# ChristophReich1996/Multi-StyleGAN

Measured on AMD Instinct MI355X. Metric: training images/sec (G+D step, 256^2, seq=3x2ch), higher is better.
Workload: dtype bf16

## Files before the change

include/msg_hip.h:

```cpp
#ifndef MSG_HIP_H
#define MSG_HIP_H

#ifdef __cplusplus
extern "C" {
#endif

enum { MSG_OK = 0, MSG_EINVAL = -1, MSG_EUNSUPPORTED = -2, MSG_ELAUNCH = -3 };
enum { MSG_F32 = 0, MSG_BF16 = 1, MSG_F16 = 2, MSG_F64 = 3, MSG_F32_SPLIT = 4 };

#define MSG_ABI_VERSION 5
int msg_abi_version(void);
const char* msg_build_arch(void);
const char* msg_strerror(int code);

int msg_upfirdn2d(const void* x, const float* fir, void* y, int dtype,
                  int major, int in_h, int in_w, int minor, int kh, int kw,
                  int up_x, int up_y, int down_x, int down_y,
                  int pad_x0, int pad_x1, int pad_y0, int pad_y1, void* stream);

int msg_upfirdn2d_pitched(const void* x, const float* fir, void* y, int dtype,
                          int major, int in_h, int in_w, int minor, int in_pitch, int kh, int kw,
                          int up_x, int up_y, int down_x, int down_y,
                          int pad_x0, int pad_x1, int pad_y0, int pad_y1, void* stream);

// ... 119 lines not shown

long long msg_minibatch_stddev_workspace(int C, int H, int W, int groups, int dtype);
int msg_minibatch_stddev(const void* x, void* y, float* stat, float* workspace, int dtype,
                         int B, int C, int H, int W, int ldx, int ldy, int groups, float alpha, void* stream);
int msg_minibatch_stddev_backward(const void* x, const void* gy, const float* gstat, void* gx, int dtype,
                                  int B, int C, int H, int W, int ldx, int ldgy, int ldgx, int groups,
                                  float alpha, void* stream);

int msg_conv2d_fprop_act(const void* x, const void* w, void* y, int dtype,
                         int B, int IH, int IW, int Cx, int Ck, int OH, int OW, int N, int ldy,
                         int kh, int kw, int stride, int pad, long long w_batch_stride,
                         const float* act_bias, const float* noise, const float* noise_weight,
                         int noise_batch, float alpha, float scale, void* stream);
int msg_conv2d_fprop_act_mask(const void* x, const void* w, void* y, int dtype,
                              int B, int IH, int IW, int Cx, int Ck, int OH, int OW, int N, int ldy,
                              int kh, int kw, int stride, int pad, long long w_batch_stride,
                              const float* act_bias, const float* noise, const float* noise_weight,
                              int noise_batch, float alpha, float scale, unsigned char* mask, void* stream);

int msg_conv2d_fprop_residual(const void* x, const void* w, void* y, int dtype,
                              int B, int IH, int IW, int Cx, int Ck, int OH, int OW, int N, int ldy,
                              int kh, int kw, int stride, int pad, long long w_batch_stride,
                              const void* residual, int res_ld, float gain, void* stream);

long long msg_conv2d_fprop_act_backward_workspace(int dtype, int B, int IH, int IW, int Cx, int Ck, int OH, int OW,
                                                  int N, int kh, int kw, long long w_batch_stride, int has_noise);
int msg_conv2d_fprop_act_backward(const void* x, const void* w, void* y, int dtype,
                                  int B, int IH, int IW, int Cx, int Ck, int OH, int OW, int N, int ldy,
                                  int kh, int kw, int stride, int pad, long long w_batch_stride,
                                  const void* residual, int res_ld,
                                  const unsigned char* sign_mask, int mask_tile_m, int mask_tile_n,
                                  const void* sign_map, int sign_ld, float alpha, float scale,
                                  float* grad_bias, const float* noise, int noise_batch, float* grad_noise_weight,
                                  float* ws, long long ws_floats, void* stream);

int msg_act_pointwise_head(const void* x, const float* bias, const float* w, float* y, int dtype,
                           long long npix, int C, float wscale, float alpha, float scale, void* stream);
long long msg_act_pointwise_head_backward_workspace(long long npix, int C);
int msg_act_pointwise_head_backward(const void* x, const float* bias, const float* w, const float* gy, void* gx,
                                    float* grad_bias_and_w, int dtype, long long npix, int C, float wscale,
                                    float alpha, float scale, float* ws, long long ws_floats, void* stream);

int msg_linear_fprop(const float* x, const float* w, const float* bias, float* y, int M, int N, int K,
                     float gain, float bias_gain, void* stream);
int msg_linear_dgrad(const float* gy, const float* w, float* gx, int M, int N, int K, float gain, void* stream);
int msg_linear_wgrad(const float* gy, const float* x, float* gw, float* gb, int M, int N, int K,
// ... 66 lines not shown
```

multi_stylegan_amd/conv_ops.py:

```python
import math
import os
from typing import Optional, Tuple

import torch
from torch.autograd import Function

from . import _lib
from ._autograd import _derive


def _vec(dtype) -> int:
    return 8 if dtype == torch.bfloat16 else 4


def _round_up(n: int, m: int) -> int:
    return (n + m - 1) // m * m


def _padded_nhwc(b, c, h, w, dtype, device):
    cx = _round_up(c, _vec(dtype))
    buf = torch.empty((b, h, w, cx), dtype=dtype, device=device)
    if cx != c:
        buf[..., c:].zero_()
    return buf.permute(0, 3, 1, 2)[:, :c]
# ... 390 lines not shown
            act_bias, noise, noise_w, alpha, scale = act[:5]
            _lib.require_gpu(x, act_bias, noise, noise_w)
            mask = None
            if len(act) > 5 and act[5] is not None and kh == 3 and stride == 1 and pad == 1:
                pkey = (x.dtype, b, ih, iw, cx, ck, oh, ow, n, kh, kw, wstride)
                mplan = _PLAN_CACHE.get(pkey)
                if mplan is None:
                    mplan = _PLAN_CACHE[pkey] = _lib.lib().msg_conv2d_fprop_plan(_lib.dtype_code(x), b, ih, iw, cx, ck, oh, ow,
                                                                                n, kh, kw, wstride)
                tile = _PLANS[mplan][1]
                if tile:
                    from .op_static.fused_act import sign_mask_for
                    mask = sign_mask_for(b, n, oh, ow, x.dtype, dev)
                    if mask is not None:
                        act[5].append((mask, tile, tile))
            code = _lib.lib().msg_conv2d_fprop_act_mask(
                xv.data_ptr(), wk.data_ptr(), y.data_ptr(), _contraction_code(x, mode), b, ih, iw, cx, ck, oh, ow, n, ldy, kh, kw,
                stride, pad, wstride, _lib.ptr(act_bias), _lib.ptr(noise), _lib.ptr(noise_w),
                1 if noise is None else noise.shape[0], float(alpha), float(scale), _lib.ptr(mask), _lib.stream_of(dev))
    _lib.check(code, "msg_conv2d_fprop")
    return y


def _grad_dest(param):
    if param is None or "_msg_grad_slot" not in getattr(param, "__dict__", ()):
        return None
    from .dist import grad_destination
    return grad_destination(param)


def wgrad_k_chunks(b, o, i, taps, oh, ow, per_sample, kp):
    tiles = ((o + 127) // 128) * ((i + 127) // 128) * taps * b
    if per_sample:
        return max(1, min((oh * ow) // (16 * kp), 1024 // tiles)) if tiles < 256 else 1
    k_chunks = max(1, min((oh * ow + 4 * kp - 1) // (4 * kp), (1024 + tiles - 1) // tiles))
    while b * k_chunks > 65535:
        k_chunks -= 1
    return k_chunks


def _launch_wgrad(gy, x, o, i, kh, kw, stride, pad, pixel_shuffle, per_sample, low_hw, raw=False, gain=1.0, out=None,
                  mode=None):
    dev = _lib.require_gpu(gy, x)
    gv, ldgy = _nhwc_view(gy)
    xv, cx = _nhwc_view(x)
    b, _, ih, iw = xv.shape
# ... 212 lines not shown
            _lib.ptr(gb), _lib.ptr(nz), nb, _lib.ptr(gnw), ws, need, _lib.stream_of(dev))
    if code == _lib.MSG_EUNSUPPORTED:
        _ACTBWD_WS_CACHE[wkey] = 0
        return None
    _lib.check(code, "msg_conv2d_fprop_act_backward")
    handle.done = (gb, gnw)
    return y


def _d_raw(gy, w, g: Geometry, residual=None, act_bwd: Optional["ActHandle"] = None, sign_map=None):
    if act_bwd is not None and act_bwd.armed and not g.per_sample and g.kind == "conv" and g.stride == 1 and g.kh == 3 and \
            g.kw == 3 and g.pad == 1 and w.ndim == 4:
        i = _oi(w)[1]
        img = _param_images(w, gy.dtype, g.wscale, g.kind)
        wk, ok = img["d"] if img is not None else \
            _cached(w, "d" + g.kind, gy.dtype, g.wscale, lambda: _relay_dgrad(w, gy.dtype, flip=True))
        out = _launch_dgrad_act_backward(gy, wk, ok, i, 3, 3, False, _oi(w)[0], act_bwd, residual=residual, mode=g.mode,
                                         sign_map=sign_map)
        if out is not None:
            return out
    return _d_raw_plain(gy, w, g, residual)


def _d_raw_plain(gy, w, g: Geometry, residual=None):
    assert residual is None or (g.kind == "conv" and g.stride == 1)
    if g.kind == "conv" and g.stride == 2 and _oi(w)[1] % _vec(gy.dtype) == 0:
        return _d_raw_s2(gy, w, g)
    i = _oi(w)[1]
    if w.ndim == 4 and _thin_ok(gy.dtype, i, g) and i <= 8 and gy.shape[1] >= 64:
        return _d_raw_thin(gy, w, g, residual)
    img = _param_images(w, gy.dtype, g.wscale, g.kind) if not g.per_sample else None
    wk, ok = img["d"] if img is not None else \
        _cached(w, "d" + g.kind, gy.dtype, g.wscale, lambda: _relay_dgrad(w, gy.dtype, flip=g.kind != "up2"))
    if g.kind == "up2":
        return _launch_fprop(gy, wk, ok, None, i, g.x_hw, 2, 2, 2, 0, 1, False, g.per_sample, _oi(w)[0], mode=g.mode)
    pad = g.kh - 1 - g.pad
    assert g.kh == g.kw
    return _launch_fprop(gy, wk, ok, None, i, g.x_hw, g.kh, g.kw, 1, pad, g.stride, False, g.per_sample, _oi(w)[0],
                         residual=residual, mode=g.mode)


def _relay_thin_dgrad(w, dtype):
    o, i, kh, kw = w.shape
    esz = 2 if dtype == torch.bfloat16 else 4
    ko, ok = 128 // esz, _round_up(o, 128 // esz)
    out = torch.zeros((ko, 1, ok), dtype=dtype, device=w.device)
# ... 152 lines not shown
            return gw.unsqueeze(0)
        return gw.reshape(oi) if w_ndim == 2 else gw

    @staticmethod
    def backward(ctx, u):
        gy, x = ctx.saved_tensors
        g = ctx.g
        ggy = _derive(_ConvF, x, u, None, g) if ctx.needs_input_grad[0] else None
        gx = _derive(_ConvD, gy, u, g) if ctx.needs_input_grad[1] else None
        return ggy, gx, None, None, None, None


class _ConvActF(Function):

    @staticmethod
    def forward(ctx, x, w, act_bias, noise, noise_w, g, alpha, scale, slot=None, out_scale=None, act_handle=None,
                input_act=None):
        o = _oi(w)[0]
        b32, nz, nw = _act_operands(act_bias, noise, noise_w, (x.shape[0], o, *g.y_hw))
        holder = [] if any(ctx.needs_input_grad) else None
        y = _f_raw(x, w, None, g, act=(b32, nz, nw, alpha, scale, holder))
        ctx.mask = holder[0] if holder else None
        ctx.slot, ctx.out_scale = slot, out_scale
        ctx.act_handle = ctx.input_act = None
        if act_handle is not None and out_scale is None and noise is None and holder is not None:
            act_handle.arm(y, ctx.mask, alpha, scale, act_bias, act_bias is not None, None)
            ctx.act_handle = act_handle if act_handle.armed else None
        if input_act is not None and input_act.armed:
            ctx.input_act = input_act
        ctx.bias_param = act_bias
        ctx.g, ctx.cfg = g, (alpha, scale, act_bias is not None, noise is not None)
        ctx.nw_shape = None if noise_w is None else noise_w.shape
        ctx.save_for_backward(x, w, y, noise)
        return y

    @staticmethod
    def backward(ctx, gy):
        from .op_static.fused_act import FusedLeakyReLUFunctionBackward
        x, w, y, noise = ctx.saved_tensors
        alpha, scale, has_bias, has_noise = ctx.cfg
        g = ctx.g
        owed = 1.0
        if ctx.out_scale is not None and ctx.out_scale.pending is not None:
            owed, ctx.out_scale.pending = ctx.out_scale.pending, None
        handed = ctx.act_handle.done if ctx.act_handle is not None else None
        if handed is not None:
            ctx.act_handle.done = None
            gpre, (gb, gnw) = gy, handed
        else:
            gpre, gb, gnw = _derive(FusedLeakyReLUFunctionBackward, gy, y, noise if has_noise else None,
                                    ctx.bias_param if has_bias else False, alpha, scale * owed, ctx.mask)
        gx = None
        if ctx.needs_input_grad[0]:
            other = ctx.slot.g if ctx.slot is not None else None
            pre = ctx.input_act if not torch.is_grad_enabled() else None
            if _dgrad_add_ok(other, x.shape, gpre.dtype, g):
                gx = _derive(_ConvD, gpre, w, g, other) if torch.is_grad_enabled() else \
                    _d_raw(gpre, w, g, residual=(other, 1.0), act_bwd=pre, sign_map=x)
                ctx.slot.merged = True
            elif pre is not None:
                gx = _d_raw(gpre, w, g, act_bwd=pre, sign_map=x)
            else:
                gx = _derive(_ConvD, gpre, w, g)
        gw = _derive(_ConvG, gpre, x, _oi(w), w.ndim, g, w) if _consumed(ctx, 1, 1) else None
        return gx, gw, (gb if has_bias and ctx.needs_input_grad[2] else None), None, \
            (gnw.reshape(ctx.nw_shape) if has_noise and ctx.needs_input_grad[4] else None), None, None, None, None, None, None, None


class _ConvResidualF(Function):

    @staticmethod
    def forward(ctx, x, w, main, g, gain, fork, slot=None, main_scale=None, out=None):
        y = _f_raw(x, w, None, g, residual=(main, gain), out=out)
        if out is not None:
            y = out.view_as(out)
        ctx.slot, ctx.main_scale = slot, main_scale
        ctx.g, ctx.gain, ctx.fork = g, float(gain), fork
        ctx.save_for_backward(x, w)
        return (y, y.view_as(y)) if fork else y

    @staticmethod
    def backward(ctx, *grads):
        from .op_static.fused_act import _ScaledAddRows, _rows_ok
        x, w = ctx.saved_tensors
        g1 = grads[0]
        g2 = grads[1] if ctx.fork else None
        if (g1 is None or g2 is None) and ctx.main_scale is not None and ctx.needs_input_grad[2]:
            gs = g1 if g1 is not None else g2
            ctx.main_scale.pending = ctx.gain
            gg = Geometry(ctx.g.kind, ctx.g.kh, ctx.g.kw, ctx.g.stride, ctx.g.pad, ctx.g.x_hw, ctx.g.per_sample,
                          ctx.g.wscale * ctx.gain, mode=ctx.g.mode)
            gs_main = gs
            if torch.is_grad_enabled() and ctx.needs_input_grad[0] and RESIDUAL_FORK_NODE:
                gx, gs_main = _ConvDFork.apply(gs, w, gg)
            else:
                gx = _derive(_ConvD, gs, w, gg) if ctx.needs_input_grad[0] else None
            if ctx.slot is not None and gx is not None:
                ctx.slot.g = gx
            gw = _derive(_ConvG, gs, x, _oi(w), w.ndim, gg, w) if _consumed(ctx, 1, 1) else None
            return gx, gw, gs_main, None, None, None, None, None, None
        if g1 is None or g2 is None:
            gs = (g1 if g1 is not None else g2) * ctx.gain
        elif _rows_ok(g1, g2):
            gs = _derive(_ScaledAddRows, g1, g2, ctx.gain)
        else:
            gs = (g1 + g2) * ctx.gain
        gx = _derive(_ConvD, gs, w, ctx.g) if ctx.needs_input_grad[0] else None
        if ctx.slot is not None and gx is not None:
            ctx.slot.g = gx
        gw = _derive(_ConvG, gs, x, _oi(w), w.ndim, ctx.g, w) if _consumed(ctx, 1, 1) else None
        return gx, gw, (gs if ctx.needs_input_grad[2] else None), None, None, None, None, None, None


class _MultiConvF(Function):

    @staticmethod
    def forward(ctx, x, geoms, *weights):
        ctx.geoms = geoms
        ctx.save_for_backward(x, *weights)
        return tuple(_f_raw(x, w, None, g) for w, g in zip(weights, geoms))

    @staticmethod
    def backward(ctx, *grads):
        x, *weights = ctx.saved_tensors
        second_order = torch.is_grad_enabled()
        gx, gws = None, []
        for k, (gy, w, g) in enumerate(zip(grads, weights, ctx.geoms)):
            if gy is None:
                gws.append(None)
                continue
# ... 3 lines not shown
                    gx = part if gx is None else gx + part
                elif second_order:
                    gx = _derive(_ConvD, gy, w, g, gx)
                else:
                    gx = _d_raw(gy, w, g, residual=(gx, 1.0))
            gws.append(_derive(_ConvG, gy, x, _oi(w), w.ndim, g, w) if _consumed(ctx, 2 + k, 1 + k) else None)
        return (gx, None, *gws)


def conv2d_shared_input(x, weights_and_scales, padding=0):
    p = _square(padding, "padding")
    geoms = tuple(Geometry("conv", w.shape[2], w.shape[3], 1, p, x.shape[2:], False, ws) for w, ws in weights_and_scales)
    return _MultiConvF.apply(x, geoms, *[w for w, _ in weights_and_scales])


class GradScale:
    __slots__ = ("pending",)

    def __init__(self):
        self.pending = None


class GradSlot:
    __slots__ = ("g", "merged")

    def __init__(self):
        self.g, self.merged = None, False


class HeadGradSlot:
    __slots__ = ("head", "dgrad", "armed")

    def __init__(self):
        self.head = None
        self.dgrad = None
        self.armed = False

    def take(self):
        head, dgrad, self.head, self.dgrad = self.head, self.dgrad, None, None
        return head, dgrad


class _ForkInput(Function):

    @staticmethod
    def forward(ctx, x, slot):
        ctx.slot = slot
        return x.view_as(x), x.view_as(x)

    @staticmethod
    def backward(ctx, g_main, g_res):
        slot = ctx.slot
        merged, slot.g, slot.merged = slot.merged, None, False
        if merged or g_res is None:
            return g_main, None
        if g_main is None:
            return g_res, None
        return g_main + g_res, None


def _square(value, what: str) -> int:
    if isinstance(value, int):
        return value
    value = tuple(value)
    if len(value) != 2 or value[0] != value[1]:
        raise _lib.MsgHipError(f"conv2d: only square {what} is implemented, got {value}")
    return int(value[0])


def fork_input(x, slot: GradSlot):
    return _ForkInput.apply(x, slot)


def conv2d_add_residual(x, weight, main, gain, stride=1, padding=0, wscale=1.0, fork=False, grad_slot=None,
                        main_grad_scale=None, out=None):
    s, p = _square(stride, "stride"), _square(padding, "padding")
# ... 670 lines not shown
```

multi_stylegan_amd/csrc/conv_dispatch.h:

```cpp
#pragma once
#include "msg_common.h"

struct ConvProblem {
    int dtype;
    int split;
    int B, IH, IW, Cx, Ck, OH, OW, N, ldy;
    int kh, kw, stride, pad, in_up, pixel_shuffle;
    long long w_batch_stride;

    bool per_sample() const { return w_batch_stride != 0; }
    int samples() const { return per_sample() ? B : 1; }
    long long mtot() const { return per_sample() ? (long long)OH * OW : (long long)B * OH * OW; }
    int esz() const { return dtype == MSG_BF16 ? 2 : 4; }
    long long x_bstride() const { return (long long)IH * IW * Cx; }
    long long y_bstride() const { return (pixel_shuffle ? 4ll : 1ll) * OH * OW * ldy; }
    long long x_bytes() const { return (long long)(per_sample() ? 1 : B) * IH * IW * Cx * esz(); }
    long long w_bytes() const { return (long long)N * kh * kw * Ck * esz(); }
    bool fits31() const { return x_bytes() < 0x7ffffff0ll && w_bytes() < 0x7ffffff0ll; }
};

enum ConvKernel {
    CONV_THIN_N, CONV_THIN_K,
    CONV_UPCONV,
    CONV_ROW3, CONV_ROW3N,
// ... 14 lines not shown
    p.B = q.B; p.IH = q.IH; p.IW = q.IW; p.Cx = q.Cx; p.Ck = q.Ck; p.OH = q.OH; p.OW = q.OW; p.N = q.N; p.ldy = q.ldy;
    p.per_sample = q.per_sample();
    if (act) p.act = *act;
    p.x_bstride = q.x_bstride();
    p.w_bstride = q.w_batch_stride;
    p.y_bstride = q.y_bstride();
    p.Mtot = (int)q.mtot();
}
template <typename P>
inline void conv_fill_taps(P& p, const ConvProblem& q) {
    p.kh = q.kh; p.kw = q.kw; p.stride = q.stride; p.pad = q.pad; p.in_up = q.in_up; p.pixel_shuffle = q.pixel_shuffle;
}

ConvPlan conv_fprop_select(const ConvProblem& q, const ActEpilogue* act, bool has_bias);

bool conv_thin_eligible(const ConvProblem& q, const ActEpilogue* act, ConvPlan* plan);
void conv_thin_launch(const ConvProblem& q, const ConvPlan& plan, const void* x, const void* w, const float* bias, void* y,
                      const ActEpilogue* act, void* stream);
bool conv_upconv_eligible(const ConvProblem& q, const ActEpilogue* act, bool has_bias, ConvPlan* plan);
void conv_upconv_launch(const ConvProblem& q, const ConvPlan& plan, const void* x, const void* w, void* y, void* stream);
bool conv_row3_eligible(const ConvProblem& q, const ActEpilogue* act, bool has_bias, ConvPlan* plan);
void conv_row3_launch(const ConvProblem& q, const ConvPlan& plan, const void* x, const void* w, const float* bias, void* y,
                      const ActEpilogue* act, void* stream);
bool conv_pp_eligible(const ConvProblem& q, ConvPlan* plan);
void conv_pp_launch(const ConvProblem& q, const ConvPlan& plan, const void* x, const void* w, const float* bias, void* y,
                    const ActEpilogue* act, void* stream);

struct WgradProblem {
    int dtype, split;
    int B, IH, IW, Cx, I, OH, OW, ldgy, O, ldgw;
    int kh, kw, stride, pad, pixel_shuffle;
    int per_sample, k_chunks, oi_major;
    float gain;
    int esz() const { return dtype == MSG_BF16 ? 2 : 4; }
    long long gy_bytes() const { return (long long)(pixel_shuffle ? 4 : 1) * OH * OW * ldgy * esz(); }
    long long x_bytes() const { return (long long)IH * IW * Cx * esz(); }
    long long slab() const { return (long long)O * kh * kw * ldgw; }
    long long gw_zstride() const { return oi_major ? (long long)O * I * kh * kw : slab(); }
};

enum WgradKernel {
    WGRAD_GENERIC, WGRAD_DMA, WGRAD_UNI,
    WGRAD_ROW3, WGRAD_ROW3_W32
};

struct WgradPlan {
// ... 27 lines not shown
```

multi_stylegan_amd/csrc/conv_fprop.hip:

```cpp
#include "conv_dispatch.h"
#include <stdlib.h>

typedef __bf16 bf16v8 __attribute__((ext_vector_type(8)));
typedef const __attribute__((address_space(1))) char* gptr_t;
typedef const __attribute__((address_space(1))) u32x4* gvec_t;
typedef __attribute__((address_space(3))) char* lds_t;

struct ConvParams {
    int B, IH, IW, Cx, Ck, OH, OW, N, ldy;
    int kh, kw, stride, pad, in_up, pixel_shuffle, per_sample;
    long long x_bstride, w_bstride, y_bstride;
    int Mtot, n_chunks, n_iters, m_tiles, n_tiles;
    ActEpilogue act;
};

constexpr int BM = 128, BN = 128, ROWB = 128;
constexpr int STAGE_BYTES = (BM + BN) * ROWB;
__device__ __attribute__((aligned(256))) unsigned int g_zero_page[16384];

__device__ __forceinline__ int swz(int row, int slot) { return row * ROWB + ((slot ^ ((row >> 1) & 7)) << 4); }

template <int SPLIT>
__device__ __forceinline__ void split_park(const u32x4& raw, char* dst) {
    uint2 pl[3];
// ... 562 lines not shown
static int conv2d_fprop_impl(const void* x, const void* w, const float* bias, void* y, const ConvProblem& q,
                             const ActEpilogue& act, void* stream, const ConvPlan* selected) {
    if (q.B == 0) return MSG_OK;
    if (!x || !w || !y || q.B < 0 || q.IH <= 0 || q.IW <= 0 || q.OH <= 0 || q.OW <= 0 || q.N <= 0 || q.kh <= 0 || q.kw <= 0 ||
        q.stride <= 0 || q.in_up <= 0 || q.Cx <= 0 || q.Ck <= 0 || q.ldy <= 0)
        return MSG_EINVAL;
    if (q.dtype != MSG_F32 && q.dtype != MSG_BF16) return MSG_EUNSUPPORTED;
    const int vec = 16 / q.esz(), bke = ROWB / q.esz();
    if (q.Ck % bke || q.Cx % vec || (((uintptr_t)x | (uintptr_t)w | (uintptr_t)y) & 15u)) return MSG_EUNSUPPORTED;
    if (q.ldy % vec || (q.pixel_shuffle && (q.N % 4 || (q.N / 4) % vec))) return MSG_EUNSUPPORTED;
    if (q.in_up > 1 && q.stride != 1) return MSG_EUNSUPPORTED;
    const ConvPlan plan = selected ? *selected : conv_fprop_select(q, &act, bias != nullptr);
    if (!plan.supported) return MSG_EUNSUPPORTED;
    switch (plan.kernel) {
        case CONV_THIN_N: case CONV_THIN_K: conv_thin_launch(q, plan, x, w, bias, y, &act, stream); break;
        case CONV_UPCONV: conv_upconv_launch(q, plan, x, w, y, stream); break;
        case CONV_ROW3: case CONV_ROW3N: conv_row3_launch(q, plan, x, w, bias, y, &act, stream); break;
        case CONV_PP: conv_pp_launch(q, plan, x, w, bias, y, &act, stream); break;
        case CONV_DMA: case CONV_REG: case CONV_REG_LEAN: case CONV_REG_SPLIT:
            conv_generic_launch(q, plan, x, w, bias, y, &act, stream); break;
    }
    return MSG_CHECK_LAUNCH();
}
```

multi_stylegan_amd/csrc/conv_fprop_row3.hip:

```cpp
#include "conv_dispatch.h"
#include <stdlib.h>
#include <type_traits>

typedef __bf16 bf16v8 __attribute__((ext_vector_type(8)));
typedef __attribute__((address_space(3))) char* lds_t;

struct ConvParamsR3 {
    int B, IH, IW, Cx, Ck, OH, OW, N, ldy;
    int per_sample, seg_len, n_seg;
    long long x_bstride, w_bstride, y_bstride;
    int Mtot, n_chunks, n_iters, m_tiles, n_tiles;
    int seg_magic;
    int ow_shift, ohw_shift;
    ActEpilogue act;
};

constexpr int HROW = 128;
constexpr int H_OOB = (int)0x80000000;

#ifdef MSG_ROW3_STAMPS
__device__ unsigned long long g_row3_stamps[256 * 4 * 3 * 8];
#define R3_STAMP(k) do { if (it >= 9 && it < 12 && L + 256 >= gridDim.x && blockIdx.z == gridDim.z - 1 && lane == 0) { unsigned long long tt; \
    asm volatile("s_memtime %0\n\ts_waitcnt lgkmcnt(0)" : "=s"(tt) :: "memory"); \
    g_row3_stamps[(((L + 256 - gridDim.x) * 4 + wid_u) * 3 + (it - 9)) * 8 + (k)] = tt; } } while (0)
extern "C" int msg_row3_debug_read(void* host_dst, int nbytes) {
    return hipMemcpyFromSymbol(host_dst, HIP_SYMBOL(g_row3_stamps), nbytes) == hipSuccess ? 0 : -1;
}
__device__ unsigned long long g_row3_clock[256 * 4 * 8];
#define R3_CLOCK(k) do { if (L + 256 >= gridDim.x && blockIdx.z == gridDim.z - 1 && lane == 0) { unsigned long long tc, tr; \
    const unsigned cl_ = L + 256 - gridDim.x; \
    asm volatile("s_memtime %0\n\ts_memrealtime %1\n\ts_waitcnt lgkmcnt(0)" : "=s"(tc), "=s"(tr) :: "memory"); \
    g_row3_clock[(cl_ * 4 + wid_u) * 8 + 2 * (k)] = tc; g_row3_clock[(cl_ * 4 + wid_u) * 8 + 2 * (k) + 1] = tr; } } while (0)
extern "C" int msg_row3_clock_read(void* host_dst, int nbytes) {
    return hipMemcpyFromSymbol(host_dst, HIP_SYMBOL(g_row3_clock), nbytes) == hipSuccess ? 0 : -1;
}
#else
#define R3_STAMP(k) do {} while (0)
#define R3_CLOCK(k) do {} while (0)
#endif

template <int MI, int NCOLB, bool S16, int EPI = 0>
__global__ __launch_bounds__(256, MI == 2 ? 2 : 1) void conv_fprop_row3_kernel(const bf16_t* __restrict__ x, const bf16_t* __restrict__ w,
                                                                 bf16_t* __restrict__ y, const float* __restrict__ bias,
                                                                 ConvParamsR3 p) {
    constexpr int VEC = 8, ESZ = 2;
    constexpr int HN = 64 * NCOLB, HB = HN * HROW, WN = 32 * NCOLB;
    constexpr int NBP = 2 * NCOLB;
    constexpr int HM = 64 * MI, WM = 32 * MI;
    constexpr int NAP = 2 * MI;
    constexpr int HA = (HM + 8) * HROW;
#if defined(MSG_ROW3_NO_STAGGER)
    constexpr bool STAGGER = false;
#else
    constexpr bool STAGGER = true;
#endif
    constexpr int EP_OFF = 2 * HA + 2 * HB;
    constexpr int SIGN_OFF = EP_OFF + (HM + HN) * 4;
    __shared__ __attribute__((aligned(16))) char smem[SIGN_OFF + (EPI == 1 ? HM * (HN / 8) : 0)];
    float* const ep_noise = reinterpret_cast<float*>(smem + EP_OFF);
    float* const ep_bias = ep_noise + HM;

    const int tid = threadIdx.x, lane = tid & 63, wid = tid >> 6;
    const int wid_u = __builtin_amdgcn_readfirstlane(wid);
    const int wm = wid_u >> 1, wn = wid_u & 1;
    constexpr int BLK = S16 ? 16 : 32;
    constexpr int NSUB = S16 ? 2 : 4, SLOTS = S16 ? 4 : 2;
    constexpr int NA = WM / BLK, NB = WN / BLK;
// ... 92 lines not shown
        if (j == NAP && wid_u != 0) return;
        lds_t la = (lds_t)(smem + abuf * HA + (j < NAP ? wid_u * (HM / 4) + 8 * j : HM) * HROW);
#if defined(__HIP_DEVICE_COMPILE__)
        __builtin_amdgcn_raw_ptr_buffer_load_lds(rs_a, la, 16, va[j], chunk * HROW, 0, 0);
#endif
    };
    auto dma_b = [&](int j, int bbuf, int tap, int chunk, bool live) __attribute__((always_inline)) {
        lds_t la = (lds_t)(smem + 2 * HA + bbuf * HB + (wid_u * (WN / 2) + 8 * j) * HROW);
#if defined(__HIP_DEVICE_COMPILE__)
        __builtin_amdgcn_raw_ptr_buffer_load_lds(rs_b, la, 16, live ? vb2[j & 1] : H_OOB,
                                                 (tap * p.n_chunks + chunk) * HROW + (j >> 1) * w_piece2, 0, 0);
#endif
    };

    typedef float accv_t __attribute__((ext_vector_type(S16 ? 4 : 16)));
    accv_t acc[NA][NB];
#pragma unroll
    for (int i = 0; i < NA; ++i)
#pragma unroll
        for (int j = 0; j < NB; ++j)
#pragma unroll
            for (int e = 0; e < (S16 ? 4 : 16); ++e) acc[i][j][e] = 0.f;

    set_kh(0);
#pragma unroll
    for (int j = 0; j < NAP + 1; ++j) dma_a(j, 0, 0);
#pragma unroll
    for (int j = 0; j < NBP; ++j) dma_b(j, 0, 0, 0, true);

    int seg_of[MI];
#pragma unroll
    for (int i = 0; i < MI; ++i) seg_of[i] = (wm * WM + i * 32) / seg;
    const int sxb = (lr >> 1) & 7;
    const int fb_base = 2 * HA + (wn * WN + lr) * HROW;

    struct Pos { int kh, chunk, kw; };
    auto k_loop = [&](auto wv_tag) __attribute__((always_inline)) {
        constexpr int WV = decltype(wv_tag)::value;
        constexpr int RPG = 3;
        constexpr int ACT_IN_FLIGHT = NAP + (WV == 0 ? 1 : 0);
        bf16v8 fa[2][NA], fb[2][NB];
        int a_addr[MI][NSUB];
        auto frag_row = [&](int i, int kw_, int buf) __attribute__((always_inline)) {
            const int r = wm * WM + i * 32 + lr + kw_ + 2 * seg_of[i];
            const int row = buf * HA + r * HROW, sx = (r >> 1) & 7;
#pragma unroll
// ... 114 lines not shown
        };
        R3_CLOCK(1);
        for (int it = 0; it < p.n_iters; it += 3) {
            k_step(std::integral_constant<int, 0>{}, it);
            k_step(std::integral_constant<int, 1>{}, it + 1);
            k_step(std::integral_constant<int, 2>{}, it + 2);
        }
        R3_CLOCK(2);
    };
    if (STAGGER) {
        switch (wid_u) {
            case 0: k_loop(std::integral_constant<int, 0>{}); break;
            case 1: k_loop(std::integral_constant<int, 1>{}); break;
            case 2: k_loop(std::integral_constant<int, 2>{}); break;
            default: k_loop(std::integral_constant<int, 3>{}); break;
        }
    } else {
        k_loop(std::integral_constant<int, -1>{});
    }
    if (S16) asm volatile("s_nop 7\n\ts_nop 7\n\ts_nop 7" ::: "memory");
    asm volatile("s_waitcnt vmcnt(0)" ::: "memory");
    __syncthreads();

    constexpr int PITCH = WN * ESZ;
    char* ep = smem + wid * (WM * PITCH);
    constexpr int G = S16 ? 1 : 4;
#pragma unroll
    for (int j = 0; j < NB; ++j)
#pragma unroll
        for (int g = 0; g < G; ++g) {
            const int unit = S16 ? 4 * j + lh : 8 * j + 2 * g + lh;
            float bv[4] = {0.f, 0.f, 0.f, 0.f};
            if (bias) {
                const int nb = n0 + wn * WN + 4 * unit;
#pragma unroll
                for (int e = 0; e < 4; ++e) bv[e] = bias[nb + e];
            }
#pragma unroll
            for (int i = 0; i < NA; ++i) {
                const int row = i * BLK + lr;
                uint2 pk;
                pk.x = (unsigned)f2bf(acc[i][j][4 * g + 0] + bv[0]) | ((unsigned)f2bf(acc[i][j][4 * g + 1] + bv[1]) << 16);
                pk.y = (unsigned)f2bf(acc[i][j][4 * g + 2] + bv[2]) | ((unsigned)f2bf(acc[i][j][4 * g + 3] + bv[3]) << 16);
                *reinterpret_cast<uint2*>(ep + row * PITCH + ((unit ^ (row & 15)) << 3)) = pk;
            }
        }
    constexpr int LPR = WN / VEC;
    constexpr int RPP = 64 / LPR;
    constexpr int NP = 64 / RPP;
    const int er = lane / LPR, u16 = lane % LPR, ec = u16 * VEC;
    const int n = n0 + wn * WN + ec;
    if constexpr (EPI == 1) {
        float cs[VEC], sn = 0.f;
#pragma unroll
        for (int e = 0; e < VEC; ++e) cs[e] = 0.f;
        const unsigned char* ep_sign = reinterpret_cast<const unsigned char*>(smem + SIGN_OFF) + (wn * WN + ec) / 8;
#pragma unroll 1
        for (int half = 0; half < MI / 2; ++half) {
            const int m_first = m0 + wm * WM + half * 64 + er;
            const long long qg = (p.per_sample ? (long long)bz * ohw : 0) + m_first;
            float a_noise[NP];
            if (p.act.noise) {
#pragma unroll
                for (int pass = 0; pass < NP; ++pass) a_noise[pass] = ep_noise[wm * WM + half * 64 + pass * RPP + er];
            }
            if (half == 0) __syncthreads();
// ... 59 lines not shown
            for (int e = 0; e < VEC; ++e) {
                float t = cs[e];
#pragma unroll
                for (int off = 32; off >= LPR; off >>= 1) t += __shfl_xor(t, off, 64);
                cs[e] = t;
            }
            if (er == 0) {
                float* dst = p.act.part_b + (mt * 2 + wm) * p.N + n;
#pragma unroll
                for (int e = 0; e < VEC; ++e) dst[e] = cs[e];
            }
        }
        if (p.act.part_n) {
            sn = wave_sum(sn);
            if (lane == 0) p.act.part_n[(mt * p.n_tiles + L % p.n_tiles) * 4 + wid] = sn;
        }
        R3_CLOCK(3);
        return;
    }
#pragma unroll 1
    for (int half = 0; half < MI / 2; ++half) {
        const int m_first = m0 + wm * WM + half * 64 + er;
        float a_bias[VEC], a_noise[NP];
        if (p.act.enabled == 1) {
#pragma unroll
            for (int e = 0; e < VEC; ++e) a_bias[e] = ep_bias[wn * WN + ec + e];
#pragma unroll
            for (int pass = 0; pass < NP; ++pass) a_noise[pass] = ep_noise[wm * WM + half * 64 + pass * RPP + er];
        }
        if (half == 0) __syncthreads();
        u32x4 v[NP];
#pragma unroll
        for (int pass = 0; pass < NP; ++pass) {
            const int row = half * 64 + pass * RPP + er;
            v[pass] = *reinterpret_cast<const u32x4*>(ep + row * PITCH + ((u16 ^ ((row & 15) >> 1)) << 4));
        }
        if (er & 1) {
#pragma unroll
            for (int pass = 0; pass < NP; ++pass) v[pass] = u32x4{v[pass][2], v[pass][3], v[pass][0], v[pass][1]};
        }
        if (p.act.enabled == 1) {
            if (p.act.alpha >= 0.f && p.act.alpha <= 1.f) {
#pragma unroll
                for (int pass = 0; pass < NP; ++pass)
                    v[pass] = act_epilogue_apply<bf16_t, true>(v[pass], a_bias, a_noise[pass], p.act.alpha, p.act.scale);
            } else {
#pragma unroll
                for (int pass = 0; pass < NP; ++pass)
                    v[pass] = act_epilogue_apply<bf16_t>(v[pass], a_bias, a_noise[pass], p.act.alpha, p.act.scale);
            }
        } else if (p.act.enabled == 2) {
            const bf16_t* rrow = reinterpret_cast<const bf16_t*>(p.act.residual) + n +
                                 ((p.per_sample ? (long long)bz * ohw : 0) + m_first) * p.act.res_ld;
            u32x4 r[NP];
#pragma unroll
            for (int pass = 0; pass < NP; ++pass)
                r[pass] = *reinterpret_cast<const u32x4*>(rrow + (long long)(pass * RPP) * p.act.res_ld);
#pragma unroll
            for (int pass = 0; pass < NP; ++pass) v[pass] = residual_epilogue_apply<bf16_t>(v[pass], r[pass], p.act.res_gain);
        }
        bf16_t* yrow = y + (p.per_sample ? (long long)bz * p.y_bstride : 0) + n + (long long)m_first * p.ldy;
#pragma unroll
        for (int pass = 0; pass < NP; ++pass) *reinterpret_cast<u32x4*>(yrow + (long long)(pass * RPP) * p.ldy) = v[pass];
        if (p.act.enabled == 1 && p.act.mask) {
            const long long tile = (long long)((p.per_sample ? (long long)bz * ohw : 0) + m0) / HM * p.n_tiles + n0 / HN;
            unsigned char* mb = p.act.mask + tile * (HM * (HN / 8)) + (wn * WN + ec) / 8 + (wm * WM + half * 64 + er) * (HN / 8);
#pragma unroll
            for (int pass = 0; pass < NP; ++pass) mb[pass * RPP * (HN / 8)] = (unsigned char)act_sign_byte(v[pass]);
        }
    }
    R3_CLOCK(3);
}

static int row3_tile_columns(int N) {
    if (N >= 256 && (long long)((N + 255) / 256) * 256 * 100 <= (long long)N * 115) return 256;
    if (N >= 128 && (long long)((N + 127) / 128) * 128 * 100 <= (long long)N * 115) return 128;
    return 0;
}

bool conv_row3_eligible(const ConvProblem& q, const ActEpilogue* act, bool has_bias, ConvPlan* plan) {
    static const int enabled = msg_tunable("MSG_CONV_ROW3", 1);
    const int IH = q.IH, IW = q.IW, Cx = q.Cx, Ck = q.Ck, OH = q.OH, OW = q.OW, N = q.N;
    if (q.dtype != MSG_BF16 || q.stride != 1 || q.pad != 1 || q.in_up != 1 || q.pixel_shuffle) return false;
    if (!enabled || q.kh != 3 || q.kw != 3 || IH != OH || IW != OW || Ck % 64 || Cx % 64) return false;
    if (conv_act_mode(act) == 3 && has_bias) return false;
    const long long mtot = q.mtot();
    static const int narrow = msg_tunable("MSG_CONV_ROW3_NARROW", 1);
    static const int w32 = msg_tunable("MSG_CONV_ROW3_W32", 1);
    int hn = row3_tile_columns(N);
    static const int shortk = msg_tunable("MSG_CONV_ROW3_SHORTK", 128);
    if (hn == 256 && Ck <= shortk && N % 128 == 0) hn = 128;
    if (OW == 32 && w32 && N >= 128 && (long long)((N + 127) / 128) * 128 * 100 <= (long long)N * 115) hn = 128;
    if (!hn || (hn == 128 && !narrow) || N % hn) return false;
    const int hm = hn;
    if (!((OW >= 64 && hm % OW == 0) || OW % hm == 0 || (OW == 32 && hm == 128))) return false;
    if (mtot < 1024 || mtot >= (1ll << 31) || mtot % hm) return false;
    if (!q.fits31()) return false;
    if ((long long)9 * (Ck / 64) * HROW >= (1ll << 24)) return false;
    const long long blocks = (mtot / hm) * ((N + hn - 1) / hn);
    if (blocks * q.samples() < (hm == 256 ? 224 : 448) || blocks >= (1ll << 31)) return false;
    const int seg_len = OW < hm ? OW : hm, seg_magic = 65536 / (seg_len + 2) + 1;
    for (int row = 0; row < hm + 16; ++row)
        if (((row * seg_magic) >> 16) != row / (seg_len + 2)) return false;
    *plan = ConvPlan{hm == 256 ? CONV_ROW3 : CONV_ROW3N, hm, hn, true};
    return true;
}

void conv_row3_launch(const ConvProblem& q, const ConvPlan& plan, const void* x, const void* w, const float* bias, void* y,
                      const ActEpilogue* act, void* stream) {
    const int hm = plan.tile_m, hn = plan.tile_n, n_chunks = q.Ck / 64;
    ConvParamsR3 p{};
    conv_fill_common(p, q, act);
    p.seg_len = q.OW < hm ? q.OW : hm;
    p.n_seg = hm / p.seg_len;
    p.n_chunks = n_chunks;
    p.n_iters = 9 * n_chunks;
    p.m_tiles = (int)(q.mtot() / hm);
    p.seg_magic = 65536 / (p.seg_len + 2) + 1;
    auto log2_exact = [](long long v) { int sh = 0; while ((1ll << sh) < v) ++sh; return (1ll << sh) == v ? sh : -1; };
    p.ow_shift = log2_exact(q.OW);
    p.ohw_shift = log2_exact((long long)q.OH * q.OW);
    if (p.ohw_shift < 0) p.ow_shift = -1;
    p.n_tiles = (q.N + hn - 1) / hn;
    dim3 grid((unsigned)((long long)p.m_tiles * p.n_tiles), 1, q.samples());
    static const int s16 = msg_tunable("MSG_CONV_ROW3_S16", 1);
    static const int s16n = msg_tunable("MSG_CONV_ROW3N_S16", 1);
#define ROW3(...) hipLaunchKernelGGL((conv_fprop_row3_kernel<__VA_ARGS__>), grid, dim3(256), 0, (hipStream_t)stream, (const bf16_t*)x, \
                                     (const bf16_t*)w, (bf16_t*)y, bias, p)
    if (p.act.enabled == 3 && hn == 256) ROW3(4, 4, true, 1);
    else if (p.act.enabled == 3) ROW3(2, 2, true, 1);
    else if (hn == 256 && s16) ROW3(4, 4, true);
    else if (hn == 256) ROW3(4, 4, false);
    else if (s16n) ROW3(2, 2, true);
    else ROW3(2, 2, false);
#undef ROW3
}
```

Measured before the change: 157.3.

## Fuse residual 1x1 skip-conv dgrad into the 3x3 row3 dgrad kernel

```diff
diff --git a/include/msg_hip.h b/include/msg_hip.h
--- a/include/msg_hip.h
+++ b/include/msg_hip.h
@@ -165,6 +165,10 @@
                               int B, int IH, int IW, int Cx, int Ck, int OH, int OW, int N, int ldy,
                               int kh, int kw, int stride, int pad, long long w_batch_stride,
                               const void* residual, int res_ld, float gain, void* stream);
+
+int msg_conv2d_fprop_side(const void* x, const void* w, void* y, int dtype,
+                          int B, int IH, int IW, int Cx, int Ck, int OH, int OW, int N, int ldy,
+                          const void* x2, int ld2, int C2, const void* w2, float gain, void* stream);
 
 long long msg_conv2d_fprop_act_backward_workspace(int dtype, int B, int IH, int IW, int Cx, int Ck, int OH, int OW,
                                                   int N, int kh, int kw, long long w_batch_stride, int has_noise);
diff --git a/multi_stylegan_amd/conv_ops.py b/multi_stylegan_amd/conv_ops.py
--- a/multi_stylegan_amd/conv_ops.py
+++ b/multi_stylegan_amd/conv_ops.py
@@ -436,6 +436,44 @@
     return y
 
 
+RESIDUAL_SIDE_DGRAD = bool(int(os.environ.get("MSG_RESIDUAL_SIDE_DGRAD", "1")))
+
+
+def _row3_tile(dtype, b, h, w_, cx, ck, n):
+    pkey = (dtype, b, h, w_, cx, ck, h, w_, n, 3, 3, 0)
+    plan = _PLAN_CACHE.get(pkey)
+    if plan is None:
+        plan = _PLAN_CACHE[pkey] = _lib.lib().msg_conv2d_fprop_plan(_lib.MSG_BF16 if dtype == torch.bfloat16 else _lib.MSG_F32,
+                                                                    b, h, w_, cx, ck, h, w_, n, 3, 3, 0)
+    return _PLANS[plan][1]
+
+
+def _launch_side(x, wk, ck, n, c_real, x2, w2k, c2, gain):
+    if x.dtype != torch.bfloat16 or x2.dtype != torch.bfloat16 or not x.is_cuda or x2.shape[1] != c2 or n % 8 or \
+            tuple(x2.shape[2:]) != tuple(x.shape[2:]) or x2.shape[0] != x.shape[0]:
+        return None
+    dev = x.device
+    xv, cx = _nhwc_view(x)
+    sv, ld2 = _nhwc_view(x2)
+    b, _, h, w_ = xv.shape
+    tile = _row3_tile(x.dtype, b, h, w_, cx, ck, n)
+    if not tile or wk.numel() < n * 9 * ck or w2k.numel() < n * c2 or not wk.is_contiguous() or not w2k.is_contiguous():
+        return None
+    y, ldy = _alloc_out(b, n, h, w_, x.dtype, dev)
+    flops = 2.0 * b * h * w_ * n * (9 * c_real + c2)
+    key = "conv_fprop_row3_side" if tile == 256 else "conv_fprop_row3n_side"
+    if _lib.kernel_clock.enabled and _CLOCK_SHAPES:
+        key += f"|B{b} {h}x{w_}->{h}x{w_} {c_real}->{n} 3x3 s1 up1 +{c2}|"
+    with _lib.on_device(dev), _lib.kernel_clock.span((key, 'bf16'), flops):
+        code = _lib.lib().msg_conv2d_fprop_side(
+            xv.data_ptr(), wk.data_ptr(), y.data_ptr(), _lib.MSG_BF16, b, h, w_, cx, ck, h, w_, n, ldy,
+            sv.data_ptr(), ld2, c2, w2k.data_ptr(), float(gain), _lib.stream_of(dev))
+    if code == _lib.MSG_EUNSUPPORTED:
+        return None
+    _lib.check(code, "msg_conv2d_fprop_side")
+    return y
+
+
 def _grad_dest(param):
     if param is None or "_msg_grad_slot" not in getattr(param, "__dict__", ()):
         return None
@@ -694,6 +732,19 @@
     return _d_raw_plain(gy, w, g, residual)
 
 
+def _d_raw_side(gy, w, g: Geometry, side):
+    gs, w_res, g_res = side
+    if g.per_sample or g.kind != "conv" or g.stride != 1 or g.kh != 3 or g.kw != 3 or g.pad != 1 or w.ndim != 4 or \
+            g_res.kind != "conv" or g_res.kh != 1 or g_res.kw != 1 or g_res.stride != 1 or g_res.pad != 0 or g_res.per_sample or \
+            gy.dtype != torch.bfloat16 or gs.dtype != torch.bfloat16 or _contraction_code(gy, g.mode) != _lib.MSG_BF16:
+        return None
+    img, img2 = _param_images(w, gy.dtype, g.wscale, g.kind), _param_images(w_res, gy.dtype, g_res.wscale, g_res.kind)
+    if img is None or img2 is None:
+        return None
+    (wk, ok), (w2k, ok2) = img["d"], img2["d"]
+    return _launch_side(gy, wk, ok, _oi(w)[1], _oi(w)[0], gs, w2k, ok2, 1.0)
+
+
 def _d_raw_plain(gy, w, g: Geometry, residual=None):
     assert residual is None or (g.kind == "conv" and g.stride == 1)
     if g.kind == "conv" and g.stride == 2 and _oi(w)[1] % _vec(gy.dtype) == 0:
@@ -892,6 +943,8 @@
         y = _f_raw(x, w, None, g, act=(b32, nz, nw, alpha, scale, holder))
         ctx.mask = holder[0] if holder else None
         ctx.slot, ctx.out_scale = slot, out_scale
+        if slot is not None:
+            slot.consumer = True
         ctx.act_handle = ctx.input_act = None
         if act_handle is not None and out_scale is None and noise is None and holder is not None:
             act_handle.arm(y, ctx.mask, alpha, scale, act_bias, act_bias is not None, None)
@@ -924,7 +977,14 @@
         if ctx.needs_input_grad[0]:
             other = ctx.slot.g if ctx.slot is not None else None
             pre = ctx.input_act if not torch.is_grad_enabled() else None
-            if _dgrad_add_ok(other, x.shape, gpre.dtype, g):
+            side = ctx.slot.take_side() if ctx.slot is not None else None
+            if side is not None:
+                gx = _d_raw_side(gpre, w, g, side) if pre is None and not torch.is_grad_enabled() else None
+                if gx is None:
+                    other = _d_raw_plain(*side)
+            if side is not None and gx is not None:
+                ctx.slot.merged = True
+            elif _dgrad_add_ok(other, x.shape, gpre.dtype, g):
                 gx = _derive(_ConvD, gpre, w, g, other) if torch.is_grad_enabled() else \
                     _d_raw(gpre, w, g, residual=(other, 1.0), act_bwd=pre, sign_map=x)
                 ctx.slot.merged = True
@@ -963,6 +1023,8 @@
             gs_main = gs
             if torch.is_grad_enabled() and ctx.needs_input_grad[0] and RESIDUAL_FORK_NODE:
                 gx, gs_main = _ConvDFork.apply(gs, w, gg)
+            elif ctx.needs_input_grad[0] and _side_handover(ctx.slot, gs, w, gg):
+                gx = None
             else:
                 gx = _derive(_ConvD, gs, w, gg) if ctx.needs_input_grad[0] else None
             if ctx.slot is not None and gx is not None:
@@ -975,7 +1037,10 @@
             gs = _derive(_ScaledAddRows, g1, g2, ctx.gain)
         else:
             gs = (g1 + g2) * ctx.gain
-        gx = _derive(_ConvD, gs, w, ctx.g) if ctx.needs_input_grad[0] else None
+        if ctx.needs_input_grad[0] and _side_handover(ctx.slot, gs, w, ctx.g):
+            gx = None
+        else:
+            gx = _derive(_ConvD, gs, w, ctx.g) if ctx.needs_input_grad[0] else None
         if ctx.slot is not None and gx is not None:
             ctx.slot.g = gx
         gw = _derive(_ConvG, gs, x, _oi(w), w.ndim, ctx.g, w) if _consumed(ctx, 1, 1) else None
@@ -1025,10 +1090,22 @@
 
 
 class GradSlot:
-    __slots__ = ("g", "merged")
+    __slots__ = ("g", "merged", "side", "consumer")
 
     def __init__(self):
-        self.g, self.merged = None, False
+        self.g, self.merged, self.side, self.consumer = None, False, None, False
+
+    def take_side(self):
+        side, self.side = self.side, None
+        return side
+
+
+def _side_handover(slot, gs, w, g) -> bool:
+    if slot is None or not slot.consumer or not RESIDUAL_SIDE_DGRAD or torch.is_grad_enabled() or gs.dtype != torch.bfloat16 or \
+            not gs.is_cuda or _oi(w)[0] % 64:
+        return False
+    slot.side = (gs, w, g)
+    return True
 
 
 class HeadGradSlot:
@@ -1055,6 +1132,9 @@
     def backward(ctx, g_main, g_res):
         slot = ctx.slot
         merged, slot.g, slot.merged = slot.merged, None, False
+        side = slot.take_side()
+        if side is not None and not merged:
+            g_res = _d_raw_plain(*side)
         if merged or g_res is None:
             return g_main, None
         if g_main is None:
diff --git a/multi_stylegan_amd/csrc/conv_dispatch.h b/multi_stylegan_amd/csrc/conv_dispatch.h
--- a/multi_stylegan_amd/csrc/conv_dispatch.h
+++ b/multi_stylegan_amd/csrc/conv_dispatch.h
@@ -60,6 +60,9 @@
 bool conv_row3_eligible(const ConvProblem& q, const ActEpilogue* act, bool has_bias, ConvPlan* plan);
 void conv_row3_launch(const ConvProblem& q, const ConvPlan& plan, const void* x, const void* w, const float* bias, void* y,
                       const ActEpilogue* act, void* stream);
+bool conv_row3_side_ok(const ConvProblem& q, int C2, int ld2);
+void conv_row3_side_launch(const ConvProblem& q, const ConvPlan& plan, const void* x, const void* w, void* y,
+                           const void* x2, int ld2, int C2, const void* w2, float gain, void* stream);
 bool conv_pp_eligible(const ConvProblem& q, ConvPlan* plan);
 void conv_pp_launch(const ConvProblem& q, const ConvPlan& plan, const void* x, const void* w, const float* bias, void* y,
                     const ActEpilogue* act, void* stream);
diff --git a/multi_stylegan_amd/csrc/conv_fprop.hip b/multi_stylegan_amd/csrc/conv_fprop.hip
--- a/multi_stylegan_amd/csrc/conv_fprop.hip
+++ b/multi_stylegan_amd/csrc/conv_fprop.hip
@@ -608,3 +608,27 @@
     }
     return MSG_CHECK_LAUNCH();
 }
+
+static int conv2d_fprop_side_impl(const void* x, const void* w, void* y, const ConvProblem& q,
+                                  const void* x2, int ld2, int C2, const void* w2, float gain, void* stream) {
+    const ActEpilogue act{};
+    if (q.B == 0) return MSG_OK;
+    if (!x || !w || !y || !x2 || !w2 || q.B < 0 || q.IH <= 0 || q.IW <= 0 || q.OH <= 0 || q.OW <= 0 || q.N <= 0 || q.Cx <= 0 ||
+        q.Ck <= 0 || q.ldy < q.N || C2 <= 0 || ld2 < C2)
+        return MSG_EINVAL;
+    if (q.dtype != MSG_BF16) return MSG_EUNSUPPORTED;
+    if (q.Ck % 64 || q.Cx % 8 || q.ldy % 8 || ld2 % 8 ||
+        (((uintptr_t)x | (uintptr_t)w | (uintptr_t)y | (uintptr_t)x2 | (uintptr_t)w2) & 15u))
+        return MSG_EUNSUPPORTED;
+    const ConvPlan plan = conv_fprop_select(q, &act, false);
+    if (!plan.supported || !is_row3(plan) || !conv_row3_side_ok(q, C2, ld2)) return MSG_EUNSUPPORTED;
+    conv_row3_side_launch(q, plan, x, w, y, x2, ld2, C2, w2, gain, stream);
+    return MSG_CHECK_LAUNCH();
+}
+
+extern "C" int msg_conv2d_fprop_side(const void* x, const void* w, void* y, int dtype,
+                                     int B, int IH, int IW, int Cx, int Ck, int OH, int OW, int N, int ldy,
+                                     const void* x2, int ld2, int C2, const void* w2, float gain, void* stream) {
+    return conv2d_fprop_side_impl(x, w, y, conv_problem(dtype, B, IH, IW, Cx, Ck, OH, OW, N, ldy, 3, 3, 1, 1, 1, 0, 0),
+                                  x2, ld2, C2, w2, gain, stream);
+}
diff --git a/multi_stylegan_amd/csrc/conv_fprop_row3.hip b/multi_stylegan_amd/csrc/conv_fprop_row3.hip
--- a/multi_stylegan_amd/csrc/conv_fprop_row3.hip
+++ b/multi_stylegan_amd/csrc/conv_fprop_row3.hip
@@ -6,6 +6,7 @@
 typedef __attribute__((address_space(3))) char* lds_t;
 
 struct ConvParamsR3 {
+    static constexpr int SIDE = 0;
     int B, IH, IW, Cx, Ck, OH, OW, N, ldy;
     int per_sample, seg_len, n_seg;
     long long x_bstride, w_bstride, y_bstride;
@@ -15,6 +16,14 @@
     ActEpilogue act;
 };
 
+struct ConvParamsR3S : ConvParamsR3 {
+    static constexpr int SIDE = 1;
+    const bf16_t* x2;
+    const bf16_t* w2;
+    int ld2, C2, side_chunks;
+    float side_gain;
+};
+
 constexpr int HROW = 128;
 constexpr int H_OOB = (int)0x80000000;
 
@@ -39,10 +48,12 @@
 #define R3_CLOCK(k) do {} while (0)
 #endif
 
-template <int MI, int NCOLB, bool S16, int EPI = 0>
+template <int MI, int NCOLB, bool S16, int EPI = 0, typename P = ConvParamsR3>
 __global__ __launch_bounds__(256, MI == 2 ? 2 : 1) void conv_fprop_row3_kernel(const bf16_t* __restrict__ x, const bf16_t* __restrict__ w,
                                                                  bf16_t* __restrict__ y, const float* __restrict__ bias,
-                                                                 ConvParamsR3 p) {
+                                                                 P p) {
+    constexpr int SIDE = P::SIDE;
+    static_assert(SIDE == 0 || (S16 && EPI == 0), "the side input: 16x16x32 MFMAs, plain epilogue");
     constexpr int VEC = 8, ESZ = 2;
     constexpr int HN = 64 * NCOLB, HB = HN * HROW, WN = 32 * NCOLB;
     constexpr int NBP = 2 * NCOLB;
@@ -181,6 +192,66 @@
 #pragma unroll
             for (int e = 0; e < (S16 ? 4 : 16); ++e) acc[i][j][e] = 0.f;
 
+    auto side_steps = [&]() __attribute__((always_inline)) {
+        if constexpr (SIDE != 0) {
+            const __amdgpu_buffer_rsrc_t rs_a2 = __builtin_amdgcn_make_buffer_rsrc((void*)p.x2, 0, 0x7ffffff0, 0x00020000);
+            const __amdgpu_buffer_rsrc_t rs_b2 = __builtin_amdgcn_make_buffer_rsrc((void*)p.w2, 0, 0x7ffffff0, 0x00020000);
+            int sa[NAP], sb[2];
+#pragma unroll
+            for (int j = 0; j < NAP; ++j) {
+                const int row = wid * (HM / 4) + 8 * j + (lane >> 3);
+                sa[j] = (int)(((long long)(m0 + row) * p.ld2 + (slot_phys ^ ((row >> 1) & 7)) * VEC) * ESZ);
+            }
+#pragma unroll
+            for (int j = 0; j < 2; ++j) {
+                const int wrow = wid * (WN / 2) + 8 * j + (lane >> 3);
+                sb[j] = (int)(((long long)(n0 + wrow) * p.C2 + (slot_phys ^ ((wrow >> 1) & 7)) * VEC) * ESZ);
+            }
+            const int w2_piece2 = 16 * p.C2 * ESZ;
+            auto stage = [&](int c) __attribute__((always_inline)) {
+                const int buf = c & 1;
+#if defined(__HIP_DEVICE_COMPILE__)
+#pragma unroll
+                for (int j = 0; j < NAP; ++j)
+                    __builtin_amdgcn_raw_ptr_buffer_load_lds(rs_a2, (lds_t)(smem + buf * HA + (wid_u * (HM / 4) + 8 * j) * HROW), 16, sa[j],
+                                                             c * HROW, 0, 0);
+#pragma unroll
+                for (int j = 0; j < NBP; ++j)
+                    __builtin_amdgcn_raw_ptr_buffer_load_lds(rs_b2, (lds_t)(smem + 2 * HA + buf * HB + (wid_u * (WN / 2) + 8 * j) * HROW), 16,
+                                                             sb[j & 1], c * HROW + (j >> 1) * w2_piece2, 0, 0);
+#endif
+            };
+            const int sx = (lr >> 1) & 7;
+            stage(0);
+#pragma unroll 1
+            for (int c = 0; c < p.side_chunks; ++c) {
+                asm volatile("s_waitcnt vmcnt(0)" ::: "memory");
+                __syncthreads();
+                if (c + 1 < p.side_chunks) stage(c + 1);
+                const char* sA = smem + (c & 1) * HA + (wm * WM + lr) * HROW;
+                const char* sB = smem + 2 * HA + (c & 1) * HB + (wn * WN + lr) * HROW;
+#pragma unroll
+                for (int sub = 0; sub < NSUB; ++sub) {
+                    const int so = ((SLOTS * sub + lh) ^ sx) << 4;
+                    bf16v8 fa[NA], fb[NB];
+#pragma unroll
+                    for (int ia = 0; ia < NA; ++ia) fa[ia] = *reinterpret_cast<const bf16v8*>(sA + ia * BLK * HROW + so);
+#pragma unroll
+                    for (int jb = 0; jb < NB; ++jb) fb[jb] = *reinterpret_cast<const bf16v8*>(sB + jb * BLK * HROW + so);
+#pragma unroll
+                    for (int ia = 0; ia < NA; ++ia)
+#pragma unroll
+                        for (int jb = 0; jb < NB; ++jb) {
+#if defined(__HIP_DEVICE_COMPILE__)
+                            asm("v_mfma_f32_16x16x32_bf16 %0, %1, %2, %0" : "+a"(acc[ia][jb]) : "v"(fb[jb]), "v"(fa[ia]));
+#endif
+                        }
+                }
+            }
+            asm volatile("s_nop 7\n\ts_nop 7\n\ts_nop 7" ::: "memory");
+            __syncthreads();
+        }
+    };
     set_kh(0);
 #pragma unroll
     for (int j = 0; j < NAP + 1; ++j) dma_a(j, 0, 0);
@@ -341,6 +412,8 @@
     asm volatile("s_waitcnt vmcnt(0)" ::: "memory");
     __syncthreads();
 
+    side_steps();
+
     constexpr int PITCH = WN * ESZ;
     char* ep = smem + wid * (WM * PITCH);
     constexpr int G = S16 ? 1 : 4;
@@ -359,8 +432,13 @@
             for (int i = 0; i < NA; ++i) {
                 const int row = i * BLK + lr;
                 uint2 pk;
+                if constexpr (SIDE != 0) {
+                    pk.x = (unsigned)f2bf(acc[i][j][4 * g + 0] * p.side_gain) | ((unsigned)f2bf(acc[i][j][4 * g + 1] * p.side_gain) << 16);
+                    pk.y = (unsigned)f2bf(acc[i][j][4 * g + 2] * p.side_gain) | ((unsigned)f2bf(acc[i][j][4 * g + 3] * p.side_gain) << 16);
+                } else {
                 pk.x = (unsigned)f2bf(acc[i][j][4 * g + 0] + bv[0]) | ((unsigned)f2bf(acc[i][j][4 * g + 1] + bv[1]) << 16);
                 pk.y = (unsigned)f2bf(acc[i][j][4 * g + 2] + bv[2]) | ((unsigned)f2bf(acc[i][j][4 * g + 3] + bv[3]) << 16);
+                }
                 *reinterpret_cast<uint2*>(ep + row * PITCH + ((unit ^ (row & 15)) << 3)) = pk;
             }
         }
@@ -466,7 +544,7 @@
     for (int half = 0; half < MI / 2; ++half) {
         const int m_first = m0 + wm * WM + half * 64 + er;
         float a_bias[VEC], a_noise[NP];
-        if (p.act.enabled == 1) {
+        if (SIDE == 0 && p.act.enabled == 1) {
 #pragma unroll
             for (int e = 0; e < VEC; ++e) a_bias[e] = ep_bias[wn * WN + ec + e];
 #pragma unroll
@@ -483,7 +561,7 @@
 #pragma unroll
             for (int pass = 0; pass < NP; ++pass) v[pass] = u32x4{v[pass][2], v[pass][3], v[pass][0], v[pass][1]};
         }
-        if (p.act.enabled == 1) {
+        if (SIDE == 0 && p.act.enabled == 1) {
             if (p.act.alpha >= 0.f && p.act.alpha <= 1.f) {
 #pragma unroll
                 for (int pass = 0; pass < NP; ++pass)
@@ -493,7 +571,7 @@
                 for (int pass = 0; pass < NP; ++pass)
                     v[pass] = act_epilogue_apply<bf16_t>(v[pass], a_bias, a_noise[pass], p.act.alpha, p.act.scale);
             }
-        } else if (p.act.enabled == 2) {
+        } else if (SIDE == 0 && p.act.enabled == 2) {
             const bf16_t* rrow = reinterpret_cast<const bf16_t*>(p.act.residual) + n +
                                  ((p.per_sample ? (long long)bz * ohw : 0) + m_first) * p.act.res_ld;
             u32x4 r[NP];
@@ -506,7 +584,7 @@
         bf16_t* yrow = y + (p.per_sample ? (long long)bz * p.y_bstride : 0) + n + (long long)m_first * p.ldy;
 #pragma unroll
         for (int pass = 0; pass < NP; ++pass) *reinterpret_cast<u32x4*>(yrow + (long long)(pass * RPP) * p.ldy) = v[pass];
-        if (p.act.enabled == 1 && p.act.mask) {
+        if (SIDE == 0 && p.act.enabled == 1 && p.act.mask) {
             const long long tile = (long long)((p.per_sample ? (long long)bz * ohw : 0) + m0) / HM * p.n_tiles + n0 / HN;
             unsigned char* mb = p.act.mask + tile * (HM * (HN / 8)) + (wn * WN + ec) / 8 + (wm * WM + half * 64 + er) * (HN / 8);
 #pragma unroll
@@ -550,10 +628,8 @@
     return true;
 }
 
-void conv_row3_launch(const ConvProblem& q, const ConvPlan& plan, const void* x, const void* w, const float* bias, void* y,
-                      const ActEpilogue* act, void* stream) {
+static void row3_fill(ConvParamsR3& p, const ConvProblem& q, const ConvPlan& plan, const ActEpilogue* act) {
     const int hm = plan.tile_m, hn = plan.tile_n, n_chunks = q.Ck / 64;
-    ConvParamsR3 p{};
     conv_fill_common(p, q, act);
     p.seg_len = q.OW < hm ? q.OW : hm;
     p.n_seg = hm / p.seg_len;
@@ -566,6 +642,33 @@
     p.ohw_shift = log2_exact((long long)q.OH * q.OW);
     if (p.ohw_shift < 0) p.ow_shift = -1;
     p.n_tiles = (q.N + hn - 1) / hn;
+}
+
+bool conv_row3_side_ok(const ConvProblem& q, int C2, int ld2) {
+    if (q.per_sample() || q.dtype != MSG_BF16 || C2 <= 0 || C2 % 64 || ld2 < C2 || ld2 % 8) return false;
+    return q.mtot() * ld2 * 2 < 0x7ffffff0ll && (long long)q.N * C2 * 2 < 0x7ffffff0ll;
+}
+
+void conv_row3_side_launch(const ConvProblem& q, const ConvPlan& plan, const void* x, const void* w, void* y,
+                           const void* x2, int ld2, int C2, const void* w2, float gain, void* stream) {
+    ConvParamsR3S p{};
+    row3_fill(p, q, plan, nullptr);
+    p.x2 = (const bf16_t*)x2; p.w2 = (const bf16_t*)w2;
+    p.ld2 = ld2; p.C2 = C2; p.side_chunks = C2 / 64; p.side_gain = gain;
+    dim3 grid((unsigned)((long long)p.m_tiles * p.n_tiles), 1, 1);
+    if (plan.tile_n == 256)
+        hipLaunchKernelGGL((conv_fprop_row3_kernel<4, 4, true, 0, ConvParamsR3S>), grid, dim3(256), 0, (hipStream_t)stream,
+                           (const bf16_t*)x, (const bf16_t*)w, (bf16_t*)y, (const float*)nullptr, p);
+    else
+        hipLaunchKernelGGL((conv_fprop_row3_kernel<2, 2, true, 0, ConvParamsR3S>), grid, dim3(256), 0, (hipStream_t)stream,
+                           (const bf16_t*)x, (const bf16_t*)w, (bf16_t*)y, (const float*)nullptr, p);
+}
+
+void conv_row3_launch(const ConvProblem& q, const ConvPlan& plan, const void* x, const void* w, const float* bias, void* y,
+                      const ActEpilogue* act, void* stream) {
+    const int hn = plan.tile_n;
+    ConvParamsR3 p{};
+    row3_fill(p, q, plan, act);
     dim3 grid((unsigned)((long long)p.m_tiles * p.n_tiles), 1, q.samples());
     static const int s16 = msg_tunable("MSG_CONV_ROW3_S16", 1);
     static const int s16n = msg_tunable("MSG_CONV_ROW3N_S16", 1);
```

After: 157.3. About the same (-0.0%).
